# oss0430/SRFRD

Hardware: NVIDIA B200
Metric: training seqs/sec; full-catalogue top-10 users/sec (higher is better)
Workload: dtype bf16

## Files before the change

include/srfrd_b200.h:

```cpp
#ifndef SRFRD_B200_H
#define SRFRD_B200_H

#include <stddef.h>
#include <stdint.h>

#ifdef __cplusplus
extern "C" {
#endif

#define SRFRD_ABI_VERSION 10
#if defined(__GNUC__)
#define SRFRD_API __attribute__((visibility("default")))
#else
#define SRFRD_API
#endif

SRFRD_API const char* srfrd_last_error(void);
SRFRD_API int srfrd_abi_version(void);
SRFRD_API int srfrd_device_check(void);

SRFRD_API int srfrd_embed_ln_fwd(const float* item_table, int64_t n_rows, int D, const float* pos_table,
                       const float* aux_table, int64_t n_aux, int F, int mode, const int64_t* seq,
                       const int64_t* aux_ids, int64_t B, int L, float item_scale, const float* ln_w,
                       const float* ln_b, float eps, void* x0_bf16, float* x0_f32, void* q_bf16, float* stats,
                       int ldx, float drop_p, uint64_t drop_seed, uint32_t drop_stream, const float* drop_step,
                       void* stream);

SRFRD_API int srfrd_srfu_labels(const int64_t* fake_ids, int64_t B, int L, int kind, int64_t* labels, void* stream);

SRFRD_API int srfrd_embed_bwd(const void* dx0_bf16, int ldx, const int64_t* seq, const int64_t* aux_ids, int64_t B, int L,
                    int D, int F, int mode, float item_scale, float* d_item, float* d_aux, void* stream);

SRFRD_API int srfrd_layernorm_fwd(const void* x_bf16, int ldx, const float* w, const float* b, float eps, void* y_bf16,
// ... 163 lines not shown
SRFRD_API int srfrd_score_loss_fused_packed(const float* h, int ldh, const float* item_table, const float* fake_table,
                                  const int64_t* pos, const int64_t* neg, const int64_t* prs, const int64_t* nrs,
                                  const float* w_pos, const float* w_neg, const float* norm, int D, int F,
                                  float* loss_acc, float* dh, int lddh, float* d_item, float* d_fake,
                                  const int* row_tok, const int* rows_dev, int64_t cap_rows, void* stream);
SRFRD_API int srfrd_embed_bwd_packed(const void* dx0_bf16, int ldx, const int64_t* seq, const int64_t* aux_ids,
                           const int* row_tok, const int* rows_dev, int64_t cap_rows, int L, int D, int F, int mode,
                           float item_scale, float* d_item, float* d_aux, float* d_pos, void* stream);

typedef struct {
  const float* bias1; const float* bias2;
  const void* gate; int ldg;
  int relu1;
  float drop1_p, drop2_p; uint32_t drop1_stream, drop2_stream; uint64_t drop_seed; const float* drop_step;
  const void* residual; int ldr;
  int residual_is_a;
  const int64_t* row_ids;
  void* mid_out; int ldm;
  void* out; int ldc;
  void* ln_out; int ld_ln; const float* ln_w; const float* ln_b; float* ln_stats; float ln_eps;
} srfrd_mlp2_t;
SRFRD_API int srfrd_mlp2_tn(const void* A_bf16, int lda, const void* W1_bf16, int ldw1, const void* W2_bf16, int ldw2, int M, int N,
                  const srfrd_mlp2_t* ep, void* stream);

SRFRD_API int srfrd_attention_live_items(const int* tok_row, int64_t B, int L, int heads, int* q_lo, int* items, int* n_live,
                               void* stream);
SRFRD_API int srfrd_set_attention_live(const int* q_lo, const int* items, const int* n_live, const int* tok_row);

typedef struct {
  const void* src; int ld_s;
  void* dst; int ld_d;
  int W;
  int mode;
} srfrd_repack_part_t;
SRFRD_API int srfrd_unpack_rows(const srfrd_repack_part_t* parts, int n_parts, const srfrd_pack_t* pk, int64_t B, int L,
                      void* stream);
SRFRD_API int srfrd_pack_rows(const srfrd_repack_part_t* parts, int n_parts, const srfrd_pack_t* pk, int64_t B, int L,
                    void* stream);

SRFRD_API int srfrd_dp_adam_step(float* const* grad_ptrs_dev, float* const* param_ptrs_dev, uint32_t* const* signal_ptrs_dev,
                       int rank, int world, int64_t n, float* m, float* v, float lr, float beta1, float beta2, float eps,
                       float* state8, const float* norm2, uint32_t* local4, void* stream, const int64_t* l2_seg,
                       int l2_n_seg, const float* l2_coef, const float* l2_reg);

#ifdef __cplusplus
}
// ... 3 lines not shown
```

srfrd_b200/_lib.py:

```python
from __future__ import annotations

import ctypes as C
import os

_HERE = os.path.dirname(os.path.abspath(__file__))
LIB_PATH = os.environ.get("SRFRD_B200_LIB") or os.path.join(_HERE, "lib", "libsrfrd_b200.so")

vp, i32, i64, f32, u32, u64 = C.c_void_p, C.c_int, C.c_int64, C.c_float, C.c_uint32, C.c_uint64


class GemmEpilogue(C.Structure):
    _fields_ = [("bias", vp), ("residual", vp), ("gate", vp), ("row_ids", vp), ("out_bf16", vp), ("out_f32", vp),
                ("ldr", i32), ("ldg", i32), ("ldc", i32), ("relu", i32), ("drop_p", f32), ("drop_stream", u32),
                ("drop_seed", u64), ("drop_step", vp),
                ("ln_out_bf16", vp), ("ln_w", vp), ("ln_b", vp), ("ln_stats", vp), ("ld_ln", i32), ("ln_eps", f32)]


class CastDesc(C.Structure):
    _fields_ = [("src", vp), ("src_ld", i32), ("dst", vp), ("dst_ld", i32), ("dst_t", vp), ("dst_t_ld", i32),
                ("rows", i32), ("cols", i32), ("dst_is_f32", i32)]


class Mlp2Epilogue(C.Structure):
    _fields_ = [("bias1", vp), ("bias2", vp), ("gate", vp), ("ldg", i32), ("relu1", i32), ("drop1_p", f32), ("drop2_p", f32),
# ... 2 lines not shown
                ("ln_out", vp), ("ld_ln", i32), ("ln_w", vp), ("ln_b", vp), ("ln_stats", vp), ("ln_eps", f32)]


class PackDesc(C.Structure):
    _fields_ = [("rows", vp), ("cnt", vp), ("seq_first", vp), ("tok_row", vp), ("row_tok", vp), ("row_ids", vp),
                ("row_info", vp), ("tile_row0", vp), ("last_row", vp), ("cap", i64)]


class RepackPart(C.Structure):
    _fields_ = [("src", vp), ("ld_s", i32), ("dst", vp), ("ld_d", i32), ("W", i32), ("mode", i32)]


SIGNATURES = {
    "srfrd_abi_version": [],
    "srfrd_device_check": [],
    "srfrd_embed_ln_fwd": [vp, i64, i32, vp, vp, i64, i32, i32, vp, vp, i64, i32, f32, vp, vp, f32, vp, vp, vp, vp, i32,
                           f32, u64, u32, vp, vp],
    "srfrd_srfu_labels": [vp, i64, i32, i32, vp, vp],
    "srfrd_embed_bwd": [vp, i32, vp, vp, i64, i32, i32, i32, i32, f32, vp, vp, vp],
    "srfrd_layernorm_fwd": [vp, i32, vp, vp, f32, vp, vp, i32, vp, i64, i32, i64, i64, vp],
    "srfrd_layernorm_bwd": [vp, vp, i32, vp, i32, vp, vp, vp, i32, vp, vp, i32, vp, vp, i64, i32, vp],
    "srfrd_gemm_tn": [vp, i32, vp, i32, i32, i32, i32, C.POINTER(GemmEpilogue), vp],
    "srfrd_mlp2_tn": [vp, i32, vp, i32, vp, i32, i32, i32, C.POINTER(Mlp2Epilogue), vp],
    "srfrd_gemm_tn_plan": [i32, i32, i32, i32, i32, i32, vp],
    "srfrd_gemm_debug_read": [vp],
    "srfrd_attn_debug_read": [vp],
    "srfrd_gemm_wgrad": [vp, i32, vp, i32, i64, i32, i32, vp, i32, vp, vp],
    "srfrd_gemm_ref": [vp, i32, vp, i32, vp, i32, i32, i32, i32, i32, i32, vp],
    "srfrd_colsum": [vp, i64, i32, i64, vp, vp],
    "srfrd_add_segments": [vp, i64, i32, i32, vp, vp],
    "srfrd_dropout_apply": [vp, i32, vp, i32, i64, i32, f32, u64, u32, vp, vp],
    "srfrd_cast_weights": [vp, i32, vp],
    "srfrd_f32_to_bf16_split": [vp, i64, vp, vp, vp, i64, i32, i32, vp],
    "srfrd_attention_fwd": [vp, i32, vp, vp, i32, vp, i32, vp, i64, i32, i32, i32, f32, u64, u32, vp, vp],
    "srfrd_attention_bwd": [vp, i32, vp, i32, vp, vp, i32, vp, i32, vp, vp, i32, vp, vp, i32, i64, i32, i32, i32, f32, u64,
                            u32, vp, vp],
    "srfrd_score_fwd": [vp, i32, vp, vp, vp, vp, vp, vp, i64, i32, i32, vp, vp, vp],
    "srfrd_score_bwd": [vp, i32, vp, vp, vp, vp, vp, vp, vp, vp, i64, i32, i32, vp, i32, vp, vp, vp],
    "srfrd_score_loss_fused": [vp, i32, vp, vp, vp, vp, vp, vp, vp, vp, vp, i64, i32, i32, vp, vp, vp, vp, i32, vp, vp, vp],
    "srfrd_weight_sums": [vp, vp, vp, i64, vp, vp],
    "srfrd_loss_finalize": [vp, vp, vp, vp],
    "srfrd_adam_tick": [vp, f32, f32, vp],
    "srfrd_adam_step": [vp, vp, vp, vp, i64, f32, f32, f32, f32, vp, i32, vp],
    "srfrd_adam_step_fused": [vp, vp, vp, vp, i64, f32, f32, f32, f32, vp, i32, vp, vp, vp, vp, vp, i32, vp, vp],
    "srfrd_param_l2_plan": [C.POINTER(i64), i32, C.POINTER(i64)],
    "srfrd_param_l2": [vp, vp, i32, i64, f32, vp, vp, vp, vp],
# ... 31 lines not shown
    "srfrd_sample_batch": [vp, vp, vp, vp, vp, i32, i32, i32, i32, i32, u64, vp, vp, vp, vp, vp, vp, vp, vp, vp, vp],
}

_lib = None
_device_ok = False
launch_count = 0


def load() -> C.CDLL:
    global _lib
    if _lib is not None:
        return _lib
    if not os.path.exists(LIB_PATH):
        raise RuntimeError(
            f"srfrd_b200: {LIB_PATH} is not built. Run `make -C srfrd_b200/csrc` (needs nvcc, sm_100a). "
            "There is no CPU fallback.")
    lib = C.CDLL(LIB_PATH)
    lib.srfrd_last_error.restype = C.c_char_p
    lib.srfrd_last_error.argtypes = []
    for name, argtypes in SIGNATURES.items():
        fn = getattr(lib, name)
        fn.argtypes = argtypes
        fn.restype = C.c_int
    if lib.srfrd_abi_version() != 10:
        raise RuntimeError("srfrd_b200: ABI version mismatch between _lib.py and the built library")
    _lib = lib
    return lib


def require_device() -> None:
    global _device_ok
    if _device_ok:
        return
    lib = load()
    if lib.srfrd_device_check() != 0:
        raise RuntimeError("srfrd_b200: " + lib.srfrd_last_error().decode())
    _device_ok = True


_profile = None


def set_profile(records) -> None:
    global _profile
    _profile = records


# ... 16 lines not shown
```

srfrd_b200/csrc/ffn.cu:

```cuda
#include <stdlib.h>

#include "common.cuh"
#include "srfrd_b200.h"

namespace srfrd {

static constexpr int MLP_THREADS = 160;
static constexpr int MT = 128;
static constexpr int MBLK = MT * 64 * 2;

struct MlpParams {
  int M, N, kb;
  int K, kbk;
  int single;
  int relu2; const bf16* gate2; int ldg2;
  const int* rows_dev;
  const float *bias1, *bias2;
  const bf16* gate; int ldg;
  int relu1;
  uint64_t drop_seed; const float* drop_step;
  uint32_t thresh1, thresh2, stream1, stream2; float scale1, scale2;
  const bf16* residual; int ldr;
  int residual_is_a;
  const int64_t* row_ids;
  const float *ln_w, *ln_b; float* ln_stats; float ln_eps; int has_ln;
};

__device__ __forceinline__ uint32_t swz_chunk(int r, int j) { return (uint32_t)(r * 128 + ((j ^ (r & 7)) << 4)); }
__device__ __forceinline__ void mlp_bar_sync() { asm volatile("bar.sync 1, 128;" ::: "memory"); }
__device__ __forceinline__ void mlp_tma_store(const CUtensorMap* tmap, const void* smem_src, int c0, int c1) {
  asm volatile("cp.async.bulk.tensor.2d.global.shared::cta.bulk_group [%0, {%2, %3}], [%1];" ::"l"(tmap),
               "r"(smem_u32(smem_src)), "r"(c0), "r"(c1)
               : "memory");
}
__device__ __forceinline__ void unpack8_bf16(const uint4& u, float* f) {
  const uint32_t w[4] = {u.x, u.y, u.z, u.w};
#pragma unroll
  for (int i = 0; i < 4; ++i) { f[2 * i] = __uint_as_float(w[i] << 16); f[2 * i + 1] = __uint_as_float(w[i] & 0xffff0000u); }
}

__global__ void __launch_bounds__(MLP_THREADS, 2)
mlp2_kernel(const __grid_constant__ CUtensorMap tmA, const __grid_constant__ CUtensorMap tmW1,
            const __grid_constant__ CUtensorMap tmW2, const __grid_constant__ CUtensorMap tmMid,
            const __grid_constant__ CUtensorMap tmOut, const __grid_constant__ CUtensorMap tmLn, MlpParams p) {
  extern __shared__ uint8_t smem_raw[];
  uint8_t* smem = reinterpret_cast<uint8_t*>((reinterpret_cast<uintptr_t>(smem_raw) + 1023) & ~uintptr_t(1023));
  const int wblk = (p.N * 128 + 1023) & ~1023;
  const int ablk = max(p.kb, p.kbk);
  uint8_t* sW1 = smem;
  uint8_t* sW2 = sW1 + p.kbk * wblk;
  uint8_t* sA = sW2 + (p.single ? 0 : p.kb) * wblk;
  uint8_t* sM = sA + ablk * MBLK;
  float* sb1 = reinterpret_cast<float*>(sM + p.kb * MBLK);
  float* sb2 = sb1 + 128;
  float* slw = sb2 + 128;
  float* slb = slw + 128;
  uint64_t* bars = reinterpret_cast<uint64_t*>(slb + 128);
  uint64_t *w_full = bars, *a_full = bars + 1, *a_free = bars + 2, *acc1_full = bars + 3, *mid_ready = bars + 4,
           *acc2_full = bars + 5;
  uint32_t* tmem_slot = reinterpret_cast<uint32_t*>(bars + 6);
  const int warp = threadIdx.x >> 5, lane = threadIdx.x & 31;

  if (warp == 4 && lane == 0) {
    tma_prefetch_desc(&tmA); tma_prefetch_desc(&tmW1); tma_prefetch_desc(&tmW2); tma_prefetch_desc(&tmMid);
    tma_prefetch_desc(&tmOut);
    if (p.has_ln) tma_prefetch_desc(&tmLn);
    mbar_init(w_full, 1); mbar_init(a_full, 1); mbar_init(a_free, 1); mbar_init(acc1_full, 1); mbar_init(mid_ready, 1);
    mbar_init(acc2_full, 1);
    fence_barrier_init();
  }
  if (warp == 4) { tmem_alloc(tmem_slot, 256); tmem_relinquish(); }
  pdl_prologue_done();
  const int M = p.rows_dev ? min(p.M, __ldg(p.rows_dev)) : p.M;
  const int n_tiles = (M + MT - 1) / MT;
  for (int i = threadIdx.x; i < 128; i += blockDim.x) {
    sb1[i] = (p.bias1 && i < p.N) ? __ldg(p.bias1 + i) : 0.f;
    sb2[i] = (p.bias2 && i < p.N) ? __ldg(p.bias2 + i) : 0.f;
    slw[i] = (p.has_ln && i < p.N) ? __ldg(p.ln_w + i) : 0.f;
    slb[i] = (p.has_ln && i < p.N) ? __ldg(p.ln_b + i) : 0.f;
  }
  tc_fence_before();
  __syncthreads();
  tc_fence_after();
  const uint32_t tmem_base = *tmem_slot;
  const uint32_t tAcc1 = tmem_base, tAcc2 = tmem_base + 128;

  if (warp == 4) {
    if ((int)blockIdx.x < n_tiles && elect_one()) {
      mbar_expect_tx(w_full, (p.kbk + (p.single ? 0 : p.kb)) * p.N * 128);
      for (int kb = 0; kb < p.kbk; ++kb) tma_load_2d(sW1 + kb * wblk, &tmW1, w_full, kb * 64, 0, SRFRD_EVICT_LAST);
      if (!p.single)
        for (int kb = 0; kb < p.kb; ++kb) tma_load_2d(sW2 + kb * wblk, &tmW2, w_full, kb * 64, 0, SRFRD_EVICT_LAST);
    }
    __syncwarp();
    const uint32_t idesc = umma_idesc_bf16(MT, p.N, 0, 0);
    const uint64_t dA = umma_smem_desc(smem_u32(sA), 0, 1024), dM = umma_smem_desc(smem_u32(sM), 0, 1024);
    const uint64_t dW1 = umma_smem_desc(smem_u32(sW1), 0, 1024), dW2 = umma_smem_desc(smem_u32(sW2), 0, 1024);
    uint32_t ph = 0;
    for (int tile = blockIdx.x; tile < n_tiles; tile += gridDim.x, ph ^= 1) {
      mbar_wait(a_free, ph ^ 1);
      if (elect_one()) {
        mbar_expect_tx(a_full, p.kbk * MBLK);
// ... 96 lines not shown
        uint4 q0 = make_uint4(0, 0, 0, 0), q1 = q0;
        if (p.gate2 && rok) {
          const uint4* gp = reinterpret_cast<const uint4*>(p.gate2 + row * p.ldg2 + c);
          q0 = __ldg(gp); q1 = __ldg(gp + 1);
        }
        tmem_ld_wait();
        float v[16], rv[16], gv2[16];
        unpack8_bf16(r0, rv); unpack8_bf16(r1, rv + 8);
        if (p.gate2) { unpack8_bf16(q0, gv2); unpack8_bf16(q1, gv2 + 8); }
#pragma unroll
        for (int i = 0; i < 16; ++i) {
          float x = __uint_as_float(raw[i]) + sb2[c + i];
          if (p.thresh2)
            x = dropout_keep(seed, p.stream2, (uint64_t)row * (uint64_t)p.N + (uint64_t)(c + i), p.thresh2) ? x * p.scale2 : 0.f;
          if (p.relu2) x = fmaxf(x, 0.f);
          if (p.gate2) x = gv2[i] > 0.f ? x : 0.f;
          x += rv[i];
          v[i] = x * rowm;
        }
        const uint4 p0 = make_uint4(pack_bf16x2(v[0], v[1]), pack_bf16x2(v[2], v[3]), pack_bf16x2(v[4], v[5]), pack_bf16x2(v[6], v[7]));
        const uint4 p1 = make_uint4(pack_bf16x2(v[8], v[9]), pack_bf16x2(v[10], v[11]), pack_bf16x2(v[12], v[13]), pack_bf16x2(v[14], v[15]));
        *reinterpret_cast<uint4*>(blk + swz_chunk(r, j)) = p0;
        *reinterpret_cast<uint4*>(blk + swz_chunk(r, j + 1)) = p1;
        if (p.has_ln) {
          float q[16];
          unpack8_bf16(p0, q); unpack8_bf16(p1, q + 8);
#pragma unroll
          for (int i = 0; i < 16; ++i) { ln_sum += q[i]; ln_sq = fmaf(q[i], q[i], ln_sq); }
        }
      }
      tc_fence_before();
      if (p.has_ln) {
        if (issuer) asm volatile("cp.async.bulk.wait_group.read 0;" ::: "memory");
        mlp_bar_sync();
        const float invn = 1.f / (float)p.N;
        const float mean = ln_sum * invn;
        const float var = fmaxf(ln_sq * invn - mean * mean, 0.f);
        const float rstd = rsqrtf(var + p.ln_eps), nb = -mean * rstd;
#pragma unroll 1
        for (int c = 0; c < p.N; c += 8) {
          const int j = (c & 63) >> 3;
          const uint4 xv = *reinterpret_cast<const uint4*>(sA + (c >> 6) * MBLK + swz_chunk(r, j));
          float q[8], y[8];
          unpack8_bf16(xv, q);
#pragma unroll
          for (int i = 0; i < 8; ++i) y[i] = fmaf(fmaf(q[i], rstd, nb), slw[c + i], slb[c + i]);
          *reinterpret_cast<uint4*>(sM + (c >> 6) * MBLK + swz_chunk(r, j)) =
              make_uint4(pack_bf16x2(y[0], y[1]), pack_bf16x2(y[2], y[3]), pack_bf16x2(y[4], y[5]), pack_bf16x2(y[6], y[7]));
        }
        if (p.ln_stats && rok) *reinterpret_cast<float2*>(p.ln_stats + 2 * row) = make_float2(mean, rstd);
      }
      fence_proxy_async();
      mlp_bar_sync();
      if (issuer) {
        for (int kb = 0; kb < p.kb; ++kb) mlp_tma_store(&tmOut, sA + kb * MBLK, kb * 64, tile * MT);
        if (p.has_ln)
          for (int kb = 0; kb < p.kb; ++kb) mlp_tma_store(&tmLn, sM + kb * MBLK, kb * 64, tile * MT);
        asm volatile("cp.async.bulk.commit_group;" ::: "memory");
        asm volatile("cp.async.bulk.wait_group.read 0;" ::: "memory");
        mbar_arrive(a_free);
      }
    }
    if (issuer) asm volatile("cp.async.bulk.wait_group 0;" ::: "memory");
  }
  tc_fence_before();
  __syncthreads();
  if (warp == 4) { tc_fence_after(); tmem_dealloc(tmem_base, 256); }
}

}

using namespace srfrd;

// ... 36 lines not shown
  if (ep->residual && ep->gate) return false;
  if (ep->ln_out_bf16 && (!ep->ln_w || !ep->ln_b || ep->ld_ln % 8 || ((uintptr_t)ep->ln_out_bf16 & 15))) return false;
  { const char* e = getenv("SRFRD_LEAN_GEMM"); if (!e || e[0] != '1') return false; }
  return row_limit() != nullptr || M <= 32768;
}
int gemm_small_launch(const void* A, int lda, const void* B, int ldb, int M, int N, int K, const srfrd_gemm_epilogue_t* ep,
                      cudaStream_t stream) {
  MlpParams p = {};
  p.M = M; p.N = N; p.K = K; p.single = 1;
  p.bias2 = ep->bias; p.relu2 = ep->relu; p.gate2 = (const bf16*)ep->gate; p.ldg2 = ep->ldg;
  p.residual = (const bf16*)ep->residual; p.ldr = ep->ldr;
  p.residual_is_a = (ep->residual == A && ep->ldr == lda && N <= K) ? 1 : 0;
  if (p.residual_is_a) p.residual = nullptr;
  p.row_ids = ep->row_ids;
  p.drop_seed = ep->drop_seed; p.drop_step = ep->drop_step; p.stream2 = ep->drop_stream;
  p.thresh2 = ep->drop_p > 0.f ? (uint32_t)((double)ep->drop_p * 4294967296.0) : 0;
  p.scale2 = ep->drop_p > 0.f ? 1.f / (1.f - ep->drop_p) : 1.f;
  p.scale1 = 1.f;
  p.ln_w = ep->ln_w; p.ln_b = ep->ln_b; p.ln_stats = ep->ln_stats; p.ln_eps = ep->ln_eps;
  return mlp_launch(p, A, lda, B, ldb, nullptr, 0, nullptr, 0, ep->out_bf16, ep->ldc, ep->ln_out_bf16, ep->ld_ln, stream);
}
}

extern "C" int srfrd_mlp2_tn(const void* A, int lda, const void* W1, int ldw1, const void* W2, int ldw2, int M, int N,
                             const srfrd_mlp2_t* ep, void* stream_) {
  cudaStream_t stream = (cudaStream_t)stream_;
  SRFRD_REQUIRE(A && W1 && W2 && ep && ep->mid_out && ep->out, "mlp2_tn: null pointer");
  SRFRD_REQUIRE(M > 0 && N >= 16 && N <= 128 && N % 16 == 0, "mlp2_tn: N = K must be a multiple of 16 up to 128 (got %d)", N);
  SRFRD_REQUIRE(lda % 8 == 0 && ldw1 % 8 == 0 && ldw2 % 8 == 0 && ep->ldm % 8 == 0 && ep->ldc % 8 == 0 && lda >= N && ldw1 >= N &&
                    ldw2 >= N && ep->ldm >= N && ep->ldc >= N, "mlp2_tn: bad leading dimensions");
  SRFRD_REQUIRE(!ep->gate || (ep->ldg % 8 == 0 && ((uintptr_t)ep->gate & 15) == 0), "mlp2_tn: bad gate");
  SRFRD_REQUIRE(!ep->residual || (ep->ldr % 8 == 0 && ((uintptr_t)ep->residual & 15) == 0), "mlp2_tn: bad residual");
  SRFRD_REQUIRE(!ep->ln_out || (ep->ln_w && ep->ln_b && ep->ld_ln % 8 == 0 && ep->ld_ln >= N), "mlp2_tn: bad LayerNorm arguments");
  SRFRD_REQUIRE(ep->drop1_p >= 0.f && ep->drop1_p < 1.f && ep->drop2_p >= 0.f && ep->drop2_p < 1.f, "mlp2_tn: dropout p must be in [0, 1)");
  MlpParams p = {};
  p.M = M; p.N = N; p.K = N; p.single = 0;
  p.bias1 = ep->bias1; p.bias2 = ep->bias2; p.gate = (const bf16*)ep->gate; p.ldg = ep->ldg; p.relu1 = ep->relu1;
  p.drop_seed = ep->drop_seed; p.drop_step = ep->drop_step; p.stream1 = ep->drop1_stream; p.stream2 = ep->drop2_stream;
  p.thresh1 = ep->drop1_p > 0.f ? (uint32_t)((double)ep->drop1_p * 4294967296.0) : 0;
  p.thresh2 = ep->drop2_p > 0.f ? (uint32_t)((double)ep->drop2_p * 4294967296.0) : 0;
  p.scale1 = ep->drop1_p > 0.f ? 1.f / (1.f - ep->drop1_p) : 1.f;
  p.scale2 = ep->drop2_p > 0.f ? 1.f / (1.f - ep->drop2_p) : 1.f;
  p.residual = (const bf16*)ep->residual; p.ldr = ep->ldr;
  p.residual_is_a = (ep->residual == nullptr && ep->residual_is_a) || (ep->residual == A && ep->ldr == lda);
  if (p.residual_is_a) p.residual = nullptr;
  p.row_ids = ep->row_ids;
  p.ln_w = ep->ln_w; p.ln_b = ep->ln_b; p.ln_stats = ep->ln_stats; p.ln_eps = ep->ln_eps;
  return mlp_launch(p, A, lda, W1, ldw1, W2, ldw2, ep->mid_out, ep->ldm, ep->out, ep->ldc, ep->ln_out, ep->ld_ln, stream);
}
```

srfrd_b200/csrc/rowwise.cu:

```cuda
#include <stdlib.h>

#include "common.cuh"
#include "srfrd_b200.h"

namespace srfrd {

static constexpr int MAXW = 512;

template <int LPR>
__device__ __forceinline__ float group_sum(float v) {
#pragma unroll
  for (int o = LPR / 2; o > 0; o >>= 1) v += __shfl_xor_sync(0xffffffffu, v, o);
  return v;
}

__device__ __forceinline__ void unpack8(const uint4& u, float* f) {
  const uint32_t w[4] = {u.x, u.y, u.z, u.w};
#pragma unroll
  for (int i = 0; i < 4; ++i) {
    const float2 t = __bfloat1622float2(*reinterpret_cast<const __nv_bfloat162*>(&w[i]));
    f[2 * i] = t.x; f[2 * i + 1] = t.y;
  }
}
__device__ __forceinline__ uint4 pack8(const float* f) {
// ... 421 lines not shown
      float xv[8], dv[8];
      unpack8(xr[ch], xv);
      if (F32DY) {
#pragma unroll
        for (int j = 0; j < 8; ++j) dv[j] = df[ch][j];
      } else {
        unpack8(dr[ch], dv);
      }
      const float4 w0 = *reinterpret_cast<const float4*>(sw + (cok ? c : 0)), w1 = *reinterpret_cast<const float4*>(sw + (cok ? c : 0) + 4);
      const float wv[8] = {w0.x, w0.y, w0.z, w0.w, w1.x, w1.y, w1.z, w1.w};
#pragma unroll
      for (int j = 0; j < 8; ++j) {
        const float xh = (cok && (!ragged || c + j < p.H)) ? (xv[j] - mean) * rstd : 0.f;
        if (ragged && c + j >= p.H) dv[j] = 0.f;
        const float g = dv[j] * wv[j];
        adw[ch][j] = fmaf(dv[j], xh, adw[ch][j]);
        adb[ch][j] += dv[j];
        sg += g;
        sgx = fmaf(g, xh, sgx);
      }
    }
    sg = group_sum<LPR>(sg) * invH;
    sgx = group_sum<LPR>(sgx) * invH;
    if (!ok) continue;
#pragma unroll
    for (int ch = 0; ch < CH; ++ch) {
      const int c = (ch * LPR + sub) * 8;
      if (c >= Hc) continue;
      float xv[8], dv[8], av[8], o[8];
      unpack8(xr[ch], xv);
      unpack8(ar[ch], av);
      if (F32DY) {
#pragma unroll
        for (int j = 0; j < 8; ++j) dv[j] = df[ch][j];
      } else {
        unpack8(dr[ch], dv);
      }
      const float4 w0 = *reinterpret_cast<const float4*>(sw + c), w1 = *reinterpret_cast<const float4*>(sw + c + 4);
      const float wv[8] = {w0.x, w0.y, w0.z, w0.w, w1.x, w1.y, w1.z, w1.w};
#pragma unroll
      for (int j = 0; j < 8; ++j) {
        const float xh = (xv[j] - mean) * rstd;
        o[j] = (rstd * (dv[j] * wv[j] - sg - xh * sgx) + av[j]) * msk;
        if (ragged && c + j >= p.H) o[j] = 0.f;
      }
      *reinterpret_cast<uint4*>(p.dx + t * p.lddx + c) = pack8(o);
    }
// ... 121 lines not shown
    float sg = 0.f, sgx = 0.f;
#pragma unroll
    for (int ch = 0; ch < CH; ++ch) {
      float xv[8], dv[8];
      unpack8(xr[ch], xv);
      if (F32DY) {
#pragma unroll
        for (int j = 0; j < 8; ++j) dv[j] = df[ch][j];
      } else {
        unpack8(dr[ch], dv);
      }
      const float4 w0 = *reinterpret_cast<const float4*>(sw + col[ch]), w1 = *reinterpret_cast<const float4*>(sw + col[ch] + 4);
      const float wv[8] = {w0.x, w0.y, w0.z, w0.w, w1.x, w1.y, w1.z, w1.w};
#pragma unroll
      for (int j = 0; j < 8; ++j) {
        const float xh = fmaf(xv[j], rstd, nb);
        const float g = dv[j] * wv[j];
        adw[ch][j] = fmaf(dv[j], xh, adw[ch][j]);
        adb[ch][j] += dv[j];
        sg += g;
        sgx = fmaf(g, xh, sgx);
      }
    }
    sg = group_sum<LPR>(sg) * invH;
    sgx = group_sum<LPR>(sgx) * invH;
#pragma unroll
    for (int ch = 0; ch < CH; ++ch) {
      float xv[8], dv[8], av[8], o[8];
      unpack8(xr[ch], xv);
      if (HAS_ADD) unpack8(ar[ch], av);
      if (F32DY) {
#pragma unroll
        for (int j = 0; j < 8; ++j) dv[j] = df[ch][j];
      } else {
        unpack8(dr[ch], dv);
      }
      const float4 w0 = *reinterpret_cast<const float4*>(sw + col[ch]), w1 = *reinterpret_cast<const float4*>(sw + col[ch] + 4);
      const float wv[8] = {w0.x, w0.y, w0.z, w0.w, w1.x, w1.y, w1.z, w1.w};
#pragma unroll
      for (int j = 0; j < 8; ++j) {
        const float xh = fmaf(xv[j], rstd, nb);
        const float u = fmaf(-sgx, xh, fmaf(dv[j], wv[j], -sg));
        o[j] = HAS_ADD ? fmaf(rstd, u, av[j]) : rstd * u;
      }
      uint4 pk = pack8(o);
      if (!keep) pk = make_uint4(0, 0, 0, 0);
// ... 239 lines not shown
  SRFRD_ROW_DISPATCH(H, CALL);
#undef CALL
  SRFRD_LAUNCH_CHECK();
  return 0;
}

extern "C" int srfrd_layernorm_fwd(const void* x, int ldx, const float* w, const float* b, float eps, void* y_bf16,
                                   float* y_f32, int ldy, float* stats, int64_t T, int H, int64_t row_stride,
                                   int64_t row_offset, void* stream) {
  return layernorm_fwd_impl(x, ldx, w, b, eps, y_bf16, y_f32, ldy, stats, T, H, row_stride, row_offset, nullptr, row_limit(),
                            stream);
}

extern "C" int srfrd_layernorm_fwd_rows(const void* x, int ldx, const float* w, const float* b, float eps, float* y_f32,
                                        int ldy, const int* row_index, int64_t n, int H, void* stream) {
  SRFRD_REQUIRE(row_index, "layernorm_fwd_rows: null row index");
  return layernorm_fwd_impl(x, ldx, w, b, eps, nullptr, y_f32, ldy, nullptr, n, H, 1, 0, row_index, nullptr, stream);
}

extern "C" int srfrd_layernorm_bwd(const void* dy_bf16, const float* dy_f32, int lddy, const void* x, int ldx,
                                   const float* stats, const float* w, const void* add, int ldadd,
                                   const int64_t* row_ids, void* dx, int lddx, float* dw, float* db, int64_t T, int H,
                                   void* stream) {
  SRFRD_REQUIRE((dy_bf16 || dy_f32) && x && stats && w && dx && dw && db, "layernorm_bwd: null pointer");
  const int Hc8 = (H + 7) & ~7;
  SRFRD_REQUIRE(H <= MAXW - 8 && ldx % 8 == 0 && lddx % 8 == 0 && lddy % 8 == 0 && (!add || ldadd % 8 == 0) &&
                    ldx >= Hc8 && lddx >= Hc8 && lddy >= Hc8 && (!add || ldadd >= Hc8),
                "layernorm_bwd: width %d / ld unsupported (rows are padded to a multiple of 8 columns)", H);
  if (T == 0) return 0;
  LnBwdParams p;
  p.dy_bf16 = (const bf16*)dy_bf16; p.dy_f32 = dy_f32; p.lddy = lddy; p.x = (const bf16*)x; p.ldx = ldx;
  p.stats = stats; p.w = w; p.add = (const bf16*)add; p.ldadd = ldadd; p.row_ids = row_ids; p.dx = (bf16*)dx;
  p.lddx = lddx; p.dw = dw; p.db = db; p.T = T; p.H = H; p.rows_dev = row_limit();
#define CALL(LPR, CH)                                                                                             \
  do {                                                                                                            \
    const int grid = grid_for_rows(T, 8 * (32 / LPR) * 8, 2);                                                     \
    if (dy_f32 && (H % 8)) SRFRD_CUDA(launch_pdl(ln_bwd_kernel<LPR, CH, true, true>, dim3(grid), dim3(256), 0, (cudaStream_t)stream, p));        \
    else if (H % 8) SRFRD_CUDA(launch_pdl(ln_bwd_kernel<LPR, CH, false, true>, dim3(grid), dim3(256), 0, (cudaStream_t)stream, p));        \
    else {                                                                                                        \
        \
      const int g3 = grid_for_rows(T, 4 * (32 / LPR) * 8, 3);                                                     \
      if (dy_f32 && add) SRFRD_CUDA(launch_pdl(ln_bwd_vec_kernel<LPR, CH, true, true, 128, 3>, dim3(g3), dim3(128), 0, (cudaStream_t)stream, p));   \
      else if (dy_f32) SRFRD_CUDA(launch_pdl(ln_bwd_vec_kernel<LPR, CH, true, false, 128, 3>, dim3(g3), dim3(128), 0, (cudaStream_t)stream, p));  \
      else if (add) SRFRD_CUDA(launch_pdl(ln_bwd_vec_kernel<LPR, CH, false, true, 128, 3>, dim3(g3), dim3(128), 0, (cudaStream_t)stream, p));     \
      else SRFRD_CUDA(launch_pdl(ln_bwd_vec_kernel<LPR, CH, false, false, 128, 3>, dim3(g3), dim3(128), 0, (cudaStream_t)stream, p));             \
    }                                                                                                             \
  } while (0)
  SRFRD_ROW_DISPATCH(H, CALL);
// ... 68 lines not shown
```

srfrd_b200/engine.py:

```python
from __future__ import annotations

import math
import os
from contextlib import contextmanager, nullcontext
from dataclasses import dataclass
from typing import Dict, List, Optional, Tuple

import torch

from . import ops

bf16 = torch.bfloat16
LN_EPS = 1e-8

KINDS = ("SRFR", "SRFRN", "SRFU_B", "SRFU_F", "SRFU_R", "SASRec")


@dataclass
class ModelSpec:
    kind: str
    item_number: int
    max_len: int
    D: int
    F: int = 0
# ... 272 lines not shown
            act(f"kv{i}", 2 * H)
            act(f"st1_{i}", 2, torch.float32)
            act(f"st2_{i}", 2, torch.float32)
            if Lmax > 128:
                ws[f"ast{i}"] = torch.zeros(T * s.num_heads, 4, dtype=torch.float32, device=dev)
        if s.kind == "SRFR":
            act("c", s.Dp)
        act("stF", 2, torch.float32)
        act("hfin", s.Doutp, torch.float32)
        act("dh", s.Doutp, torch.float32)
        for n in ("gA", "gC", "gD", "gX"):
            act(n)
        for i in range(nb):
            for n in ("gda1_", "gdr_", "gdq_"):
                act(f"{n}{i}")
            act(f"gdz_{i}")
            act(f"gdkv_{i}", 2 * H)
        if s.kind == "SRFR":
            act("gc", s.Dp)
        if s.dropout > 0:
            for i in range(nb):
                act(f"gE_{i}")
        ws["pos_tmp"] = torch.zeros(Lmax * H, dtype=torch.float32, device=dev)
        self._ws, self._ws_tokens = ws, T
        self.ws_generation += 1
        return ws

    def packed_ok(self, B: int, L: int) -> bool:
        return self.packed_mode(B, L) is not None

    def packed_mode(self, B: int, L: int) -> Optional[str]:
        s = self.spec
        if s.padded or s.H % 16 or s.D % 8 or B > 16384 or B < 1:
            return None
        if ops.attention_packed_supported(L, s.H, s.num_heads):
            return "tile"
        if self.hybrid and L <= 4096:
            return "hybrid"
        return None

    def _hybrid_ws(self, Td: int) -> Dict[str, torch.Tensor]:
        hw = getattr(self, "_hws", None)
        if hw is not None and hw["_rows"] >= Td:
            return hw
        s, dev = self.spec, self.device
        Hp = s.Hp
        hw = {"_rows": Td}
        z = lambda w: torch.zeros(Td, w, dtype=bf16, device=dev)
        for i in range(s.num_blocks):
# ... 140 lines not shown

    def check_saved(self, version: Optional[int] = None) -> "_Saved":
        sv = self.saved
        if sv is None and version is None:
            raise RuntimeError("backward() without a training forward()")
        if sv is None or sv.version != self.fwd_version or (version is not None and version != sv.version):
            raise RuntimeError("srfrd_b200: backward() of a stale forward -- another forward() (training, validation or "
                               "predict) ran on this model after the one being back-propagated and overwrote the shared "
                               "activation workspace; run backward() before the next forward()")
        return sv

    def backward(self, dh: torch.Tensor, version: Optional[int] = None) -> None:
        s, P = self.spec, self.P
        sv = self.check_saved(version)
        T, H, Hp, nb = sv.T, s.H, s.Hp, s.num_blocks
        ws = self._ws
        row_ids = sv.row_ids
        p_drop, seed, step = sv.p_drop, sv.seed, sv.step
        gA, gC, gD, gX = (ws[n][:T] for n in ("gA", "gC", "gD", "gX"))
        G = lambda name: P.view(name, grad=True)
        GM = lambda name: P.mat(name, grad=True)
        x = [ws[f"x{i}"][:T] for i in range(nb + 1)]
        dz_top = ws[f"gdz_{nb - 1}"][:T]
        with ops.row_limit(sv.plan.rows) if sv.plan is not None else nullcontext():
            if s.kind == "SRFR":
                gc = ws["gc"][:T]
                ops.layernorm_bwd(dh, ws["c"][:T], ws["stF"][:T], P.view("last_layernorm.weight"), gc,
                                  G("last_layernorm.weight"), G("last_layernorm.bias"), H=s.D)
                with self._branch():
                    ops.gemm_wgrad(gc, x[nb], GM("last_conv.weight"), G("last_conv.bias"), Mo=s.D, No=H)
                ops.gemm_tn(gc, self.sh["wcT"], out_bf16=dz_top, row_ids=row_ids)
            else:
                ops.layernorm_bwd(dh, x[nb], ws["stF"][:T], P.view("last_layernorm.weight"), dz_top,
                                  G("last_layernorm.weight"), G("last_layernorm.bias"), row_ids=row_ids, H=s.Dout)

            for i in reversed(range(nb)):
                Q, q, kv, o, r, y, h1 = (ws[f"{n}{i}"][:T] for n in ("Q", "q", "kv", "o", "r", "y", "h1"))
                dz, da1, dr, dq, dkv = (ws[f"{n}{i}"][:T] for n in ("gdz_", "gda1_", "gdr_", "gdq_", "gdkv_"))
                dx_out = ws[f"gdz_{i - 1}"][:T] if i > 0 else gA
                dz2 = dz
                if p_drop > 0:
                    dz2 = ws[f"gE_{i}"][:T]
                    ops.dropout_apply(dz, dz2, Hp, p_drop, seed, 12 + 4 * i, step)
                with self._branch():
                    ops.gemm_wgrad(dz2, h1, GM(f"forward_layers.{i}.conv2.weight"), G(f"forward_layers.{i}.conv2.bias"),
                                   Mo=H, No=H)
                if sv.mlp2:
                    ops.mlp2_tn(dz2, self.sh[f"w2T{i}"], self.sh[f"w1T{i}"], da1, gC, gate=h1, drop1_p=p_drop,
                                drop1_stream=11 + 4 * i, drop_seed=seed, drop_step=step, residual=dz)
                else:
                    ops.gemm_tn(dz2, self.sh[f"w2T{i}"], out_bf16=da1, gate=h1, drop_p=p_drop, drop_seed=seed,
                                drop_stream=11 + 4 * i, drop_step=step)
                with self._branch():
                    ops.gemm_wgrad(da1, y, GM(f"forward_layers.{i}.conv1.weight"), G(f"forward_layers.{i}.conv1.bias"),
                                   Mo=H, No=H)
                if not sv.mlp2:
                    ops.gemm_tn(da1, self.sh[f"w1T{i}"], out_bf16=gC, residual=dz)
                ops.layernorm_bwd(gC, r, ws[f"st2_{i}"][:T], P.view(f"forward_layernorms.{i}.weight"), dr,
                                  G(f"forward_layernorms.{i}.weight"), G(f"forward_layernorms.{i}.bias"), H=H)
                with self._branch():
                    ops.gemm_wgrad(dr, o, GM(f"attention_layers.{i}.out_proj.weight"),
                                   G(f"attention_layers.{i}.out_proj.bias"), Mo=H, No=H)
                if not sv.oproj & 2:
                    ops.gemm_tn(dr, self.sh[f"woT{i}"], out_bf16=gC)
                self._attention_bwd(sv, i, gC, q, kv, o, dq, dkv, dr, ws.get(f"ast{i}"))
                gin = GM(f"attention_layers.{i}.in_proj_weight")
                gbin = G(f"attention_layers.{i}.in_proj_bias")
                with self._branch():
                    ops.gemm_wgrad(dq, Q, gin[:H], gbin[:H], Mo=H, No=H)
                    if Hp == H:
                        ops.gemm_wgrad(dkv, x[i], gin[H:], gbin[H:], Mo=2 * H, No=H)
                    else:
                        ops.gemm_wgrad(dkv[:, :Hp], x[i], gin[H:2 * H], gbin[H:2 * H], Mo=H, No=H)
                        ops.gemm_wgrad(dkv[:, Hp:], x[i], gin[2 * H:], gbin[2 * H:], Mo=H, No=H)
                with self._branch(second=True):
                    ops.gemm_tn(dkv, self.sh[f"wkvT{i}"], out_bf16=gX)
                ops.gemm_tn(dq, self.sh[f"wqT{i}"], out_bf16=gD, residual=dr)
                self._join(second=True)
                ops.layernorm_bwd(gD, x[i], ws[f"st1_{i}"][:T], P.view(f"attention_layernorms.{i}.weight"), dx_out,
                                  G(f"attention_layernorms.{i}.weight"), G(f"attention_layernorms.{i}.bias"),
                                  add=gX, row_ids=row_ids, H=H)
            dx0 = gA
# ... 45 lines not shown
```

srfrd_b200/ops.py:

```python
from __future__ import annotations

import ctypes as C
from typing import Optional

import torch

from . import _lib
from contextlib import contextmanager

from ._lib import CastDesc, GemmEpilogue, Mlp2Epilogue, PackDesc, RepackPart, call

bf16 = torch.bfloat16


def _p(t: Optional[torch.Tensor]):
    return None if t is None else t.data_ptr()


def _stream():
    return torch.cuda.current_stream().cuda_stream


def _chk(t: torch.Tensor, dtype, name: str):
    if not t.is_cuda:
# ... 26 lines not shown


def embed_bwd(dx0, seq, aux_ids, D, F, mode, item_scale, d_item, d_aux):
    B, L = seq.shape
    call("srfrd_embed_bwd", _p(dx0), dx0.stride(0), _p(seq), _p(aux_ids), B, L, D, F, mode, float(item_scale),
         _p(d_item), _p(d_aux), _stream())


def layernorm_fwd(x, w, b, eps, y_bf16=None, y_f32=None, stats=None, T=None, H=None, row_stride=1, row_offset=0):
    _lib.require_device()
    T = x.shape[0] if T is None else T
    H = x.shape[1] if H is None else H
    y = y_bf16 if y_bf16 is not None else y_f32
    call("srfrd_layernorm_fwd", _p(x), x.stride(0), _p(w), _p(b), float(eps), _p(y_bf16), _p(y_f32), y.stride(0),
         _p(stats), T, H, row_stride, row_offset, _stream())


def layernorm_bwd(dy, x, stats, w, dx, dw, db, add=None, row_ids=None, H=None):
    T = x.shape[0]
    H = x.shape[1] if H is None else H
    dyb = dy if dy.dtype == bf16 else None
    dyf = dy if dy.dtype == torch.float32 else None
    call("srfrd_layernorm_bwd", _p(dyb), _p(dyf), dy.stride(0), _p(x), x.stride(0), _p(stats), _p(w), _p(add),
         0 if add is None else add.stride(0), _p(row_ids), _p(dx), dx.stride(0), _p(dw), _p(db), T, H, _stream())


def gemm_tn(A, B, out_bf16=None, out_f32=None, bias=None, residual=None, gate=None, row_ids=None, relu=False,
            drop_p=0.0, drop_seed=0, drop_stream=0, drop_step=None, M=None, ln_out=None, ln_w=None, ln_b=None, ln_eps=0.0,
            ln_stats=None):
    _lib.require_device()
    M = A.shape[0] if M is None else M
    K = A.shape[1]
    N = B.shape[0]
    out = out_bf16 if out_bf16 is not None else out_f32
    ep = GemmEpilogue(_p(bias), _p(residual), _p(gate), _p(row_ids), _p(out_bf16), _p(out_f32),
                      0 if residual is None else residual.stride(0), 0 if gate is None else gate.stride(0),
                      out.stride(0), int(relu), float(drop_p), int(drop_stream), int(drop_seed), _p(drop_step),
                      _p(ln_out), _p(ln_w), _p(ln_b), _p(ln_stats), 0 if ln_out is None else ln_out.stride(0), float(ln_eps))
    call("srfrd_gemm_tn", _p(A), A.stride(0), _p(B), B.stride(0), M, N, K, C.byref(ep), _stream())


def gemm_wgrad(dY, X, dW, dbias=None, Mo=None, No=None):
    T = dY.shape[0]
    Mo = dY.shape[1] if Mo is None else Mo
    No = X.shape[1] if No is None else No
    call("srfrd_gemm_wgrad", _p(dY), dY.stride(0), _p(X), X.stride(0), T, Mo, No, _p(dW), dW.stride(0), _p(dbias),
         _stream())
# ... 325 lines not shown


def _parts(parts):
    arr = (RepackPart * len(parts))()
    for i, (src, dst, W, mode) in enumerate(parts):
        arr[i] = RepackPart(_p(src), src.stride(0), _p(dst), dst.stride(0), int(W), int(mode))
    return arr


def unpack_rows(parts, plan: PackedPlan):
    _lib.require_device()
    arr = _parts(parts)
    call("srfrd_unpack_rows", arr, len(parts), C.byref(plan.desc), plan.B, plan.L, _stream())


def pack_rows(parts, plan: PackedPlan):
    _lib.require_device()
    arr = _parts(parts)
    call("srfrd_pack_rows", arr, len(parts), C.byref(plan.desc), plan.B, plan.L, _stream())


def mlp2_tn(A, W1, W2, mid_out, out, bias1=None, bias2=None, gate=None, relu1=False, drop1_p=0.0, drop2_p=0.0, drop1_stream=0,
            drop2_stream=0, drop_seed=0, drop_step=None, residual=None, residual_is_a=False, row_ids=None, ln_out=None,
            ln_w=None, ln_b=None, ln_stats=None, ln_eps=0.0, M=None):
    _lib.require_device()
    M = A.shape[0] if M is None else M
    N = W1.shape[0]
    ep = Mlp2Epilogue(_p(bias1), _p(bias2), _p(gate), 0 if gate is None else gate.stride(0), int(relu1), float(drop1_p),
                      float(drop2_p), int(drop1_stream), int(drop2_stream), int(drop_seed), _p(drop_step), _p(residual),
                      0 if residual is None else residual.stride(0), int(residual_is_a), _p(row_ids), _p(mid_out),
                      mid_out.stride(0), _p(out), out.stride(0), _p(ln_out), 0 if ln_out is None else ln_out.stride(0),
                      _p(ln_w), _p(ln_b), _p(ln_stats), float(ln_eps))
    call("srfrd_mlp2_tn", _p(A), A.stride(0), _p(W1), W1.stride(0), _p(W2), W2.stride(0), M, N, C.byref(ep), _stream())


def catalogue_ce_plan(Dp: int):
    smem, stages, tmem = C.c_int64(0), C.c_int(0), C.c_int(0)
    call("srfrd_catalogue_ce_plan", int(Dp), C.byref(smem), C.byref(stages), C.byref(tmem))
    return int(smem.value), int(stages.value), int(tmem.value)


def _ce_rows(h, plan):
    return (None, None, h.shape[0]) if plan is None else (plan.row_tok, plan.rows, plan.cap)


def catalogue_ce_fwd(h, table, pos, w_pos, lse, loss_acc, plan: Optional[PackedPlan] = None):
    _lib.require_device()
    _chk(h, bf16, "h"); _chk(table, bf16, "table"); _chk(pos, torch.int64, "pos")
    row_tok, rows, cap = _ce_rows(h, plan)
    call("srfrd_catalogue_ce_fwd", _p(h), h.stride(0), _p(table), table.stride(0), table.shape[0] - 1, table.shape[1],
         _p(pos), _p(w_pos), _p(row_tok), _p(rows), cap, _p(lse), _p(loss_acc), _stream())


def catalogue_ce_bwd(h, table, pos, w_pos, norm, lse, dh, d_item, D, plan: Optional[PackedPlan] = None):
    _lib.require_device()
    _chk(h, bf16, "h"); _chk(table, bf16, "table"); _chk(pos, torch.int64, "pos")
# ... 5 lines not shown
```

Measured before the change: 9.831 million.

## Fold LayerNorm backward dx into fused FFN backward kernel epilogue

After: 9.403 million, median of 6. -4.4%, worse.

```diff
diff --git a/include/srfrd_b200.h b/include/srfrd_b200.h
--- a/include/srfrd_b200.h
+++ b/include/srfrd_b200.h
@@ -8,7 +8,7 @@
 extern "C" {
 #endif
 
-#define SRFRD_ABI_VERSION 10
+#define SRFRD_ABI_VERSION 11
 #if defined(__GNUC__)
 #define SRFRD_API __attribute__((visibility("default")))
 #else
@@ -218,6 +218,8 @@
 } srfrd_mlp2_t;
 SRFRD_API int srfrd_mlp2_tn(const void* A_bf16, int lda, const void* W1_bf16, int ldw1, const void* W2_bf16, int ldw2, int M, int N,
                   const srfrd_mlp2_t* ep, void* stream);
+SRFRD_API int srfrd_mlp2_tn_ln_bwd(const void* A_bf16, int lda, const void* W1_bf16, int ldw1, const void* W2_bf16, int ldw2,
+                  int M, int N, const srfrd_mlp2_t* ep, const void* x_bf16, int ldx, void* stream);
 
 SRFRD_API int srfrd_attention_live_items(const int* tok_row, int64_t B, int L, int heads, int* q_lo, int* items, int* n_live,
                                void* stream);
diff --git a/srfrd_b200/_lib.py b/srfrd_b200/_lib.py
--- a/srfrd_b200/_lib.py
+++ b/srfrd_b200/_lib.py
@@ -48,6 +48,7 @@
     "srfrd_layernorm_bwd": [vp, vp, i32, vp, i32, vp, vp, vp, i32, vp, vp, i32, vp, vp, i64, i32, vp],
     "srfrd_gemm_tn": [vp, i32, vp, i32, i32, i32, i32, C.POINTER(GemmEpilogue), vp],
     "srfrd_mlp2_tn": [vp, i32, vp, i32, vp, i32, i32, i32, C.POINTER(Mlp2Epilogue), vp],
+    "srfrd_mlp2_tn_ln_bwd": [vp, i32, vp, i32, vp, i32, i32, i32, C.POINTER(Mlp2Epilogue), vp, i32, vp],
     "srfrd_gemm_tn_plan": [i32, i32, i32, i32, i32, i32, vp],
     "srfrd_gemm_debug_read": [vp],
     "srfrd_attn_debug_read": [vp],
@@ -125,7 +126,7 @@
         fn = getattr(lib, name)
         fn.argtypes = argtypes
         fn.restype = C.c_int
-    if lib.srfrd_abi_version() != 10:
+    if lib.srfrd_abi_version() != 11:
         raise RuntimeError("srfrd_b200: ABI version mismatch between _lib.py and the built library")
     _lib = lib
     return lib
diff --git a/srfrd_b200/csrc/ffn.cu b/srfrd_b200/csrc/ffn.cu
--- a/srfrd_b200/csrc/ffn.cu
+++ b/srfrd_b200/csrc/ffn.cu
@@ -24,6 +24,7 @@
   int residual_is_a;
   const int64_t* row_ids;
   const float *ln_w, *ln_b; float* ln_stats; float ln_eps; int has_ln;
+  const bf16* ln_x; int ldlx;
 };
 
 __device__ __forceinline__ uint32_t swz_chunk(int r, int j) { return (uint32_t)(r * 128 + ((j ^ (r & 7)) << 4)); }
@@ -37,6 +38,64 @@
   const uint32_t w[4] = {u.x, u.y, u.z, u.w};
 #pragma unroll
   for (int i = 0; i < 4; ++i) { f[2 * i] = __uint_as_float(w[i] << 16); f[2 * i + 1] = __uint_as_float(w[i] & 0xffff0000u); }
+}
+
+template <int LPR, int CH>
+__device__ __forceinline__ void mlp_ln_bwd_row(const MlpParams& p, int r, int64_t row, bool rok, const uint8_t* sA,
+                                               uint8_t* sM, const float* slw) {
+  if (!rok) {
+    for (int c = 0; c < p.N; c += 8)
+      *reinterpret_cast<uint4*>(sM + (c >> 6) * MBLK + swz_chunk(r, (c & 63) >> 3)) = make_uint4(0, 0, 0, 0);
+    return;
+  }
+  const float2 st = __ldg(reinterpret_cast<const float2*>(p.ln_stats + 2 * row));
+  const float rstd = st.y, nb = -st.x * st.y;
+  const bf16* xrow = p.ln_x + row * p.ldlx;
+  float sg[LPR], sgx[LPR];
+#pragma unroll
+  for (int s = 0; s < LPR; ++s) {
+    sg[s] = 0.f; sgx[s] = 0.f;
+#pragma unroll
+    for (int ch = 0; ch < CH; ++ch) {
+      const int c = (ch * LPR + s) * 8;
+      if (c >= p.N) continue;
+      float xv[8], dv[8];
+      unpack8_bf16(__ldg(reinterpret_cast<const uint4*>(xrow + c)), xv);
+      unpack8_bf16(*reinterpret_cast<const uint4*>(sA + (c >> 6) * MBLK + swz_chunk(r, (c & 63) >> 3)), dv);
+#pragma unroll
+      for (int j = 0; j < 8; ++j) {
+        const float xh = fmaf(xv[j], rstd, nb);
+        const float g = __fmul_rn(dv[j], slw[c + j]);
+        sg[s] += g;
+        sgx[s] = fmaf(g, xh, sgx[s]);
+      }
+    }
+  }
+#pragma unroll
+  for (int o = LPR / 2; o > 0; o >>= 1) {
+    float t[LPR], tx[LPR];
+#pragma unroll
+    for (int s = 0; s < LPR; ++s) { t[s] = sg[s] + sg[s ^ o]; tx[s] = sgx[s] + sgx[s ^ o]; }
+#pragma unroll
+    for (int s = 0; s < LPR; ++s) { sg[s] = t[s]; sgx[s] = tx[s]; }
+  }
+  const float invH = 1.f / (float)p.N;
+  const float msg = sg[0] * invH, msgx = sgx[0] * invH;
+#pragma unroll 1
+  for (int c = 0; c < p.N; c += 8) {
+    uint8_t* chunk = sM + (c >> 6) * MBLK + swz_chunk(r, (c & 63) >> 3);
+    float xv[8], dv[8], o[8];
+    unpack8_bf16(__ldg(reinterpret_cast<const uint4*>(xrow + c)), xv);
+    unpack8_bf16(*reinterpret_cast<const uint4*>(sA + (c >> 6) * MBLK + swz_chunk(r, (c & 63) >> 3)), dv);
+#pragma unroll
+    for (int j = 0; j < 8; ++j) {
+      const float xh = fmaf(xv[j], rstd, nb);
+      const float u = fmaf(-msgx, xh, fmaf(dv[j], slw[c + j], -msg));
+      o[j] = rstd * u;
+    }
+    *reinterpret_cast<uint4*>(chunk) =
+        make_uint4(pack_bf16x2(o[0], o[1]), pack_bf16x2(o[2], o[3]), pack_bf16x2(o[4], o[5]), pack_bf16x2(o[6], o[7]));
+  }
 }
 
 __global__ void __launch_bounds__(MLP_THREADS, 2)
@@ -77,7 +136,7 @@
     sb1[i] = (p.bias1 && i < p.N) ? __ldg(p.bias1 + i) : 0.f;
     sb2[i] = (p.bias2 && i < p.N) ? __ldg(p.bias2 + i) : 0.f;
     slw[i] = (p.has_ln && i < p.N) ? __ldg(p.ln_w + i) : 0.f;
-    slb[i] = (p.has_ln && i < p.N) ? __ldg(p.ln_b + i) : 0.f;
+    slb[i] = (p.ln_b && i < p.N) ? __ldg(p.ln_b + i) : 0.f;
   }
   tc_fence_before();
   __syncthreads();
@@ -220,7 +279,7 @@
         const uint4 p1 = make_uint4(pack_bf16x2(v[8], v[9]), pack_bf16x2(v[10], v[11]), pack_bf16x2(v[12], v[13]), pack_bf16x2(v[14], v[15]));
         *reinterpret_cast<uint4*>(blk + swz_chunk(r, j)) = p0;
         *reinterpret_cast<uint4*>(blk + swz_chunk(r, j + 1)) = p1;
-        if (p.has_ln) {
+        if (p.has_ln && !p.ln_x) {
           float q[16];
           unpack8_bf16(p0, q); unpack8_bf16(p1, q + 8);
 #pragma unroll
@@ -231,6 +290,12 @@
       if (p.has_ln) {
         if (issuer) asm volatile("cp.async.bulk.wait_group.read 0;" ::: "memory");
         mlp_bar_sync();
+        if (p.ln_x) {
+          if (p.N <= 32) mlp_ln_bwd_row<4, 1>(p, r, row, rok, sA, sM, slw);
+          else if (p.N <= 64) mlp_ln_bwd_row<8, 1>(p, r, row, rok, sA, sM, slw);
+          else if (p.N <= 96) mlp_ln_bwd_row<4, 3>(p, r, row, rok, sA, sM, slw);
+          else mlp_ln_bwd_row<16, 1>(p, r, row, rok, sA, sM, slw);
+        } else {
         const float invn = 1.f / (float)p.N;
         const float mean = ln_sum * invn;
         const float var = fmaxf(ln_sq * invn - mean * mean, 0.f);
@@ -247,6 +312,7 @@
               make_uint4(pack_bf16x2(y[0], y[1]), pack_bf16x2(y[2], y[3]), pack_bf16x2(y[4], y[5]), pack_bf16x2(y[6], y[7]));
         }
         if (p.ln_stats && rok) *reinterpret_cast<float2*>(p.ln_stats + 2 * row) = make_float2(mean, rstd);
+        }
       }
       fence_proxy_async();
       mlp_bar_sync();
@@ -329,8 +395,8 @@
 }
 }
 
-extern "C" int srfrd_mlp2_tn(const void* A, int lda, const void* W1, int ldw1, const void* W2, int ldw2, int M, int N,
-                             const srfrd_mlp2_t* ep, void* stream_) {
+static int mlp2_impl(const void* A, int lda, const void* W1, int ldw1, const void* W2, int ldw2, int M, int N,
+                     const srfrd_mlp2_t* ep, const void* ln_x, int ldx, void* stream_) {
   cudaStream_t stream = (cudaStream_t)stream_;
   SRFRD_REQUIRE(A && W1 && W2 && ep && ep->mid_out && ep->out, "mlp2_tn: null pointer");
   SRFRD_REQUIRE(M > 0 && N >= 16 && N <= 128 && N % 16 == 0, "mlp2_tn: N = K must be a multiple of 16 up to 128 (got %d)", N);
@@ -338,7 +404,9 @@
                     ldw2 >= N && ep->ldm >= N && ep->ldc >= N, "mlp2_tn: bad leading dimensions");
   SRFRD_REQUIRE(!ep->gate || (ep->ldg % 8 == 0 && ((uintptr_t)ep->gate & 15) == 0), "mlp2_tn: bad gate");
   SRFRD_REQUIRE(!ep->residual || (ep->ldr % 8 == 0 && ((uintptr_t)ep->residual & 15) == 0), "mlp2_tn: bad residual");
-  SRFRD_REQUIRE(!ep->ln_out || (ep->ln_w && ep->ln_b && ep->ld_ln % 8 == 0 && ep->ld_ln >= N), "mlp2_tn: bad LayerNorm arguments");
+  SRFRD_REQUIRE(!ep->ln_out || (ep->ln_w && (ep->ln_b || ln_x) && ep->ld_ln % 8 == 0 && ep->ld_ln >= N), "mlp2_tn: bad LayerNorm arguments");
+  SRFRD_REQUIRE(!ln_x || (ep->ln_out && ep->ln_stats && ldx % 8 == 0 && ldx >= N && ((uintptr_t)ln_x & 15) == 0),
+                "mlp2_tn: bad LayerNorm backward arguments");
   SRFRD_REQUIRE(ep->drop1_p >= 0.f && ep->drop1_p < 1.f && ep->drop2_p >= 0.f && ep->drop2_p < 1.f, "mlp2_tn: dropout p must be in [0, 1)");
   MlpParams p = {};
   p.M = M; p.N = N; p.K = N; p.single = 0;
@@ -352,6 +420,18 @@
   p.residual_is_a = (ep->residual == nullptr && ep->residual_is_a) || (ep->residual == A && ep->ldr == lda);
   if (p.residual_is_a) p.residual = nullptr;
   p.row_ids = ep->row_ids;
-  p.ln_w = ep->ln_w; p.ln_b = ep->ln_b; p.ln_stats = ep->ln_stats; p.ln_eps = ep->ln_eps;
+  p.ln_w = ep->ln_w; p.ln_b = ln_x ? nullptr : ep->ln_b; p.ln_stats = ep->ln_stats; p.ln_eps = ep->ln_eps;
+  p.ln_x = (const bf16*)ln_x; p.ldlx = ldx;
   return mlp_launch(p, A, lda, W1, ldw1, W2, ldw2, ep->mid_out, ep->ldm, ep->out, ep->ldc, ep->ln_out, ep->ld_ln, stream);
 }
+
+extern "C" int srfrd_mlp2_tn(const void* A, int lda, const void* W1, int ldw1, const void* W2, int ldw2, int M, int N,
+                             const srfrd_mlp2_t* ep, void* stream) {
+  return mlp2_impl(A, lda, W1, ldw1, W2, ldw2, M, N, ep, nullptr, 0, stream);
+}
+
+extern "C" int srfrd_mlp2_tn_ln_bwd(const void* A, int lda, const void* W1, int ldw1, const void* W2, int ldw2, int M, int N,
+                                    const srfrd_mlp2_t* ep, const void* ln_x, int ldx, void* stream) {
+  SRFRD_REQUIRE(ln_x, "mlp2_tn_ln_bwd: null LayerNorm input");
+  return mlp2_impl(A, lda, W1, ldw1, W2, ldw2, M, N, ep, ln_x, ldx, stream);
+}
diff --git a/srfrd_b200/csrc/rowwise.cu b/srfrd_b200/csrc/rowwise.cu
--- a/srfrd_b200/csrc/rowwise.cu
+++ b/srfrd_b200/csrc/rowwise.cu
@@ -467,7 +467,7 @@
     }
     sg = group_sum<LPR>(sg) * invH;
     sgx = group_sum<LPR>(sgx) * invH;
-    if (!ok) continue;
+    if (!ok || !p.dx) continue;
 #pragma unroll
     for (int ch = 0; ch < CH; ++ch) {
       const int c = (ch * LPR + sub) * 8;
@@ -635,6 +635,7 @@
         sgx = fmaf(g, xh, sgx);
       }
     }
+    if (!p.dx) continue;
     sg = group_sum<LPR>(sg) * invH;
     sgx = group_sum<LPR>(sgx) * invH;
 #pragma unroll
@@ -920,8 +921,9 @@
                                    const float* stats, const float* w, const void* add, int ldadd,
                                    const int64_t* row_ids, void* dx, int lddx, float* dw, float* db, int64_t T, int H,
                                    void* stream) {
-  SRFRD_REQUIRE((dy_bf16 || dy_f32) && x && stats && w && dx && dw && db, "layernorm_bwd: null pointer");
+  SRFRD_REQUIRE((dy_bf16 || dy_f32) && x && stats && w && dw && db, "layernorm_bwd: null pointer");
   const int Hc8 = (H + 7) & ~7;
+  if (!dx) { add = nullptr; row_ids = nullptr; lddx = Hc8; }
   SRFRD_REQUIRE(H <= MAXW - 8 && ldx % 8 == 0 && lddx % 8 == 0 && lddy % 8 == 0 && (!add || ldadd % 8 == 0) &&
                     ldx >= Hc8 && lddx >= Hc8 && lddy >= Hc8 && (!add || ldadd >= Hc8),
                 "layernorm_bwd: width %d / ld unsupported (rows are padded to a multiple of 8 columns)", H);
diff --git a/srfrd_b200/engine.py b/srfrd_b200/engine.py
--- a/srfrd_b200/engine.py
+++ b/srfrd_b200/engine.py
@@ -318,9 +318,17 @@
             for i in range(nb):
                 act(f"gE_{i}")
         ws["pos_tmp"] = torch.zeros(Lmax * H, dtype=torch.float32, device=dev)
+        if self._ln2_foldable():
+            for i in range(nb):
+                act(f"gdy_{i}")
         self._ws, self._ws_tokens = ws, T
         self.ws_generation += 1
         return ws
+
+    def _ln2_foldable(self) -> bool:
+        s = self.spec
+        return (self.overlap and self.fuse_ffn and self.fuse_ln and s.H == s.Hp <= 128
+                and ops.attention_packed_supported(s.max_len, s.H, s.num_heads))
 
     def packed_ok(self, B: int, L: int) -> bool:
         return self.packed_mode(B, L) is not None
@@ -507,6 +515,7 @@
         GM = lambda name: P.mat(name, grad=True)
         x = [ws[f"x{i}"][:T] for i in range(nb + 1)]
         dz_top = ws[f"gdz_{nb - 1}"][:T]
+        ln2_fold = sv.mlp2 and sv.hyb is None and self._ln2_foldable()
         with ops.row_limit(sv.plan.rows) if sv.plan is not None else nullcontext():
             if s.kind == "SRFR":
                 gc = ws["gc"][:T]
@@ -530,9 +539,12 @@
                 with self._branch():
                     ops.gemm_wgrad(dz2, h1, GM(f"forward_layers.{i}.conv2.weight"), G(f"forward_layers.{i}.conv2.bias"),
                                    Mo=H, No=H)
+                ln2_w = P.view(f"forward_layernorms.{i}.weight")
+                dy = ws[f"gdy_{i}"][:T] if ln2_fold else gC
                 if sv.mlp2:
-                    ops.mlp2_tn(dz2, self.sh[f"w2T{i}"], self.sh[f"w1T{i}"], da1, gC, gate=h1, drop1_p=p_drop,
-                                drop1_stream=11 + 4 * i, drop_seed=seed, drop_step=step, residual=dz)
+                    fold = dict(ln_out=dr, ln_x=r, ln_w=ln2_w, ln_stats=ws[f"st2_{i}"][:T]) if ln2_fold else {}
+                    ops.mlp2_tn(dz2, self.sh[f"w2T{i}"], self.sh[f"w1T{i}"], da1, dy, gate=h1, drop1_p=p_drop,
+                                drop1_stream=11 + 4 * i, drop_seed=seed, drop_step=step, residual=dz, **fold)
                 else:
                     ops.gemm_tn(dz2, self.sh[f"w2T{i}"], out_bf16=da1, gate=h1, drop_p=p_drop, drop_seed=seed,
                                 drop_stream=11 + 4 * i, drop_step=step)
@@ -541,8 +553,13 @@
                                    Mo=H, No=H)
                 if not sv.mlp2:
                     ops.gemm_tn(da1, self.sh[f"w1T{i}"], out_bf16=gC, residual=dz)
-                ops.layernorm_bwd(gC, r, ws[f"st2_{i}"][:T], P.view(f"forward_layernorms.{i}.weight"), dr,
-                                  G(f"forward_layernorms.{i}.weight"), G(f"forward_layernorms.{i}.bias"), H=H)
+                ln2 = (dy, r, ws[f"st2_{i}"][:T], ln2_w)
+                ln2_g = (G(f"forward_layernorms.{i}.weight"), G(f"forward_layernorms.{i}.bias"))
+                if ln2_fold:
+                    with self._branch():
+                        ops.layernorm_bwd(*ln2, None, *ln2_g, H=H)
+                else:
+                    ops.layernorm_bwd(*ln2, dr, *ln2_g, H=H)
                 with self._branch():
                     ops.gemm_wgrad(dr, o, GM(f"attention_layers.{i}.out_proj.weight"),
                                    G(f"attention_layers.{i}.out_proj.bias"), Mo=H, No=H)
diff --git a/srfrd_b200/ops.py b/srfrd_b200/ops.py
--- a/srfrd_b200/ops.py
+++ b/srfrd_b200/ops.py
@@ -72,7 +72,8 @@
     dyb = dy if dy.dtype == bf16 else None
     dyf = dy if dy.dtype == torch.float32 else None
     call("srfrd_layernorm_bwd", _p(dyb), _p(dyf), dy.stride(0), _p(x), x.stride(0), _p(stats), _p(w), _p(add),
-         0 if add is None else add.stride(0), _p(row_ids), _p(dx), dx.stride(0), _p(dw), _p(db), T, H, _stream())
+         0 if add is None else add.stride(0), _p(row_ids), _p(dx), 0 if dx is None else dx.stride(0), _p(dw), _p(db), T, H,
+         _stream())
 
 
 def gemm_tn(A, B, out_bf16=None, out_f32=None, bias=None, residual=None, gate=None, row_ids=None, relu=False,
@@ -444,7 +445,7 @@
 
 def mlp2_tn(A, W1, W2, mid_out, out, bias1=None, bias2=None, gate=None, relu1=False, drop1_p=0.0, drop2_p=0.0, drop1_stream=0,
             drop2_stream=0, drop_seed=0, drop_step=None, residual=None, residual_is_a=False, row_ids=None, ln_out=None,
-            ln_w=None, ln_b=None, ln_stats=None, ln_eps=0.0, M=None):
+            ln_w=None, ln_b=None, ln_stats=None, ln_eps=0.0, M=None, ln_x=None):
     _lib.require_device()
     M = A.shape[0] if M is None else M
     N = W1.shape[0]
@@ -453,7 +454,11 @@
                       0 if residual is None else residual.stride(0), int(residual_is_a), _p(row_ids), _p(mid_out),
                       mid_out.stride(0), _p(out), out.stride(0), _p(ln_out), 0 if ln_out is None else ln_out.stride(0),
                       _p(ln_w), _p(ln_b), _p(ln_stats), float(ln_eps))
-    call("srfrd_mlp2_tn", _p(A), A.stride(0), _p(W1), W1.stride(0), _p(W2), W2.stride(0), M, N, C.byref(ep), _stream())
+    if ln_x is None:
+        call("srfrd_mlp2_tn", _p(A), A.stride(0), _p(W1), W1.stride(0), _p(W2), W2.stride(0), M, N, C.byref(ep), _stream())
+    else:
+        call("srfrd_mlp2_tn_ln_bwd", _p(A), A.stride(0), _p(W1), W1.stride(0), _p(W2), W2.stride(0), M, N, C.byref(ep),
+             _p(ln_x), ln_x.stride(0), _stream())
 
 
 def catalogue_ce_plan(Dp: int):
```
